# kmjc/PulsePortraiture

Measured on AMD Instinct MI355X. Metric: TOAs/sec (phase+DM fit, 64ch×2048bin fp64) at 1/2/4/8 MI355X, higher is better.
Workload: dtype f64

## Files before the change

pulseportraiture_amd/csrc/ppfit_capi_fit.hip:

```cpp
#include "ppfit_host.hpp"

namespace {

int taylor_lds_moments(ppf_ctx* ctx, int nchan, size_t lds_meta) {
  if (ctx->taylor_static_lds == kUnknown) {
    size_t mx = 0;
    const void* ks[4] = {reinterpret_cast<const void*>(&k_fit_taylor<true, false>),
                         reinterpret_cast<const void*>(&k_fit_taylor<false, false>),
                         reinterpret_cast<const void*>(&k_fit_taylor<true, true>),
                         reinterpret_cast<const void*>(&k_fit_taylor<false, true>)};
    for (const void* k : ks) {
      hipFuncAttributes at;
      if (hipFuncGetAttributes(&at, k) != hipSuccess) return 0;
      mx = std::max(mx, at.sharedSizeBytes);
    }
    ctx->taylor_static_lds = mx;
  }
  const size_t stat = ctx->taylor_static_lds;
  const size_t per_block = (kLdsPerCU / kTaylorBlocksPerCU) & ~(size_t)1023;
  if (per_block <= stat + lds_meta) return 0;
  const size_t nl = (per_block - stat - lds_meta) / ((size_t)nchan * sizeof(double));
  return (int)std::min<size_t>(nl, kMT);
}

int sync_event(ppf_ctx* ctx, size_t i, hipEvent_t* out) {
  while (ctx->sync_events.size() <= i) {
    hipEvent_t e;
    HIPCHK(ctx, hipEventCreateWithFlags(&e, hipEventDisableTiming));
    ctx->sync_events.push_back(e);
  }
  *out = ctx->sync_events[i];
  return PPF_OK;
}


struct FitWorkspace : WsPlan {
  int X, R, sig, dsum, st, acc, wsc, T, G;

  FitWorkspace(int nchan, int NHP, bool taylor, bool wide, int64_t ws_limit, int64_t nsub) {
    const size_t bR = (size_t)NHP * sizeof(double2);
    const size_t bC = (size_t)nchan * sizeof(double);
    X = array((size_t)nchan * NHP * sizeof(double2));
    R = array(bR);
    array(bR);
    sig = array(bC);
    dsum = array(bC);
    st = array(sizeof(SolveState));
    acc = array((size_t)2 * nchan * 10 * sizeof(double));
    wsc = array((size_t)nchan * 8 * sizeof(double));
    T = array(taylor ? (size_t)2 * nchan * kMT * sizeof(double) : 0);
    G = array(wide ? align256(std::max(meta_lds(nchan), xspec_dyn_lds(nchan))) : 0);
    lay_out(nsub, ws_limit, 1024);
  }

  void slice(int sub, SpecArgs& sa, FitArgs& fa) const {
    fa.X = sa.X = at<double2>(X, sub);
    fa.R = sa.R = at<double2>(R, sub);
    fa.sig = sa.sig = at<double>(sig, sub);
    fa.dsum = sa.dsum = at<double>(dsum, sub);
    fa.st = at<SolveState>(st, sub);
    fa.acc = at<double>(acc, sub);
    fa.wsc = at<double>(wsc, sub);
    fa.T = per[T] ? at<double>(T, sub) : nullptr;
    fa.gdyn = sa.gdyn = per[G] ? at<unsigned char>(G, sub) : nullptr;
    fa.gdyn_stride = sa.gdyn_stride = per[G];
  }
};

struct FitLaunch {
  int logN, nbin;
  bool wide;
  size_t lds_meta;
  size_t lds_xspec, lds_guess, lds_taylor, lds_scat;
};


int stage_data(ppf_ctx* ctx, hipStream_t st, int n, const SpecArgs& sa, const FitLaunch& L) {
  const int nbin = L.nbin;
  return timed_on(ctx, PPF_K_DATA_XSPEC, st, [&] {
    if (L.logN < 0) {
      const int nrows = n * sa.nchan, NH = nbin / 2 + 1;
      const double* rows = sa.data + (size_t)sa.sub0 * sa.nchan * nbin;
      const dim3 g((nrows + kGenRows - 1) / kGenRows, (NH + 255) / 256);
      double2* dst = sa.D ? sa.D : sa.X;
      if (sa.spec_mode != PPF_SPEC_USE) {
        if (nbin <= kGenLdsTw)
          hipLaunchKernelGGL(k_dft_rows_mfma<true>, g, dim3(kBlock), dft_mfma_lds(nbin, true), st,
                             rows, dst, nrows, nbin, sa.NHP, sa.tw);
        else
          hipLaunchKernelGGL(k_dft_rows_mfma<false>, g, dim3(kBlock), dft_mfma_lds(nbin, false),
                             st, rows, dst, nrows, nbin, sa.NHP, sa.tw);
      }
      hipLaunchKernelGGL(k_data_post_gen, dim3(n), dim3(kBlock), 0, st, sa, nbin);
    }
    LOGN_SWITCH(L.logN, WIDE_SWITCH(L.wide, hipLaunchKernelGGL((k_data_xspec<LG, WD>), dim3(n),
                                                               dim3(XspecCfg<LG>::WPB * 64),
                                                               L.lds_xspec, st, sa)));
  });
}

int stage_guess(ppf_ctx* ctx, hipStream_t st, int n, const FitArgs& fa, const FitLaunch& L) {
  return timed_on(ctx, PPF_K_GUESS, st, [&] {
    if (fa.guess && fa.guess_wave) hipLaunchKernelGGL(k_guess_w, dim3(n), dim3(64), 0, st, fa);
    hipLaunchKernelGGL(k_guess, dim3(n), dim3(kBlock), fa.guess ? L.lds_guess : 0, st, fa);
  });
}

int stage_moments(ppf_ctx* ctx, hipStream_t st, int n, const FitArgs& fa) {
  if (ctx->opt[PPF_OPT_FUSE_MOMENTS]) return PPF_OK;
  return timed_on(ctx, PPF_K_MOMENTS, st, [&] {
    const dim3 g(n, (fa.nchan + 16 * kWaves - 1) / (16 * kWaves));
    if (fa.Dsp) hipLaunchKernelGGL((k_moments<4, true>), g, dim3(kBlock), 0, st, fa);
    else hipLaunchKernelGGL((k_moments<4, false>), g, dim3(kBlock), 0, st, fa);
  });
}

int stage_taylor(ppf_ctx* ctx, hipStream_t st, int n, const FitArgs& fa, const FitLaunch& L) {
  const bool mom = ctx->opt[PPF_OPT_FUSE_MOMENTS] != 0;
  const dim3 g(n), b(kBlock);
  const size_t lds = L.lds_taylor;
  return timed_on(ctx, PPF_K_FIT_TAYLOR, st, [&] {
    WIDE_SWITCH(L.wide, {
      if (fa.Dsp) {
        if (mom) hipLaunchKernelGGL((k_fit_taylor<true, true, WD>), g, b, lds, st, fa);
        else hipLaunchKernelGGL((k_fit_taylor<false, true, WD>), g, b, lds, st, fa);
      } else {
        if (mom) hipLaunchKernelGGL((k_fit_taylor<true, false, WD>), g, b, lds, st, fa);
        else hipLaunchKernelGGL((k_fit_taylor<false, false, WD>), g, b, lds, st, fa);
      }
    });
  });
}

int stage_post(ppf_ctx* ctx, hipStream_t st, int n, const FitArgs& fa, const FitLaunch& L) {
  return timed_on(ctx, PPF_K_POST, st, [&] {
    if (post_wave_ok(fa)) hipLaunchKernelGGL(k_post_w, dim3(n), dim3(64), L.lds_meta, st, fa);
    WIDE_SWITCH(L.wide, {
      if (!post_wave_ok(fa))
        hipLaunchKernelGGL((k_post<false, WD>), dim3(n), dim3(kBlock), L.lds_meta, st, fa);
      hipLaunchKernelGGL((k_post<true, WD>), dim3(n), dim3(kBlock), L.lds_meta, st, fa);
    });
  });
}

int stage_errs(ppf_ctx* ctx, hipStream_t st, int n, const SpecArgs& sa, double* errs_out) {
  if (!errs_out) return PPF_OK;
  HIPCHK(ctx, hipMemcpyAsync(errs_out + (size_t)sa.sub0 * sa.nchan, sa.sig,
                             (size_t)n * sa.nchan * sizeof(double), hipMemcpyDeviceToDevice, st));
  return PPF_OK;
}

int scat_split_solve(ppf_ctx* ctx, const FitArgs& fa, int nc, int split, size_t lds_scat) {
  const int nchan = fa.nchan;
  double* part = static_cast<double*>(ctx->buf[kSpart].p);
  int* ctrs = reinterpret_cast<int*>(part + (size_t)nc * ((nchan + 7) / 8) * kScatPart);
  HIPCHK(ctx, hipMemsetAsync(ctrs, 0, 2 * sizeof(int), ctx->stream));
  constexpr int kCheck = 4;
  int cur = split;
  const int split_tail = std::max(split, std::min(32, (nchan + 31) / 32));
  hipGraphExec_t gx[2] = {nullptr, nullptr};
  auto graph_for = [&](int sp, hipGraphExec_t* ex) -> int {
    if (*ex) return PPF_OK;
    if (!ctx->stream2)
      HIPCHK(ctx, hipStreamCreateWithFlags(&ctx->stream2, hipStreamNonBlocking));
    hipStream_t cs = ctx->stream2;
    hipGraph_t g = nullptr;
    HIPCHK(ctx, hipStreamBeginCapture(cs, hipStreamCaptureModeThreadLocal));
    for (int k = 0; k < kCheck; ++k) {
      hipLaunchKernelGGL(k_scat_sweep, dim3(nc, sp), dim3(kBlock), lds_scat, cs, fa, part, sp, 0);
      hipLaunchKernelGGL(k_scat_step, dim3(nc), dim3(64), 0, cs, fa, part, 0, ctrs, k & 1);
    }
    HIPCHK(ctx, hipStreamEndCapture(cs, &g));
    const hipError_t e = hipGraphInstantiate(ex, g, nullptr, nullptr, 0);
    (void)hipGraphDestroy(g);
    if (e != hipSuccess)
      return fail(ctx, PPF_ERR_DEVICE, "scattering solve graph: %s", hipGetErrorString(e));
    return PPF_OK;
  };
  struct GraphFree {
    hipGraphExec_t* g;
    hipStream_t st;
    ~GraphFree() {
      if (!g[0] && !g[1]) return;
      (void)hipStreamSynchronize(st);
      for (int i = 0; i < 2; ++i)
        if (g[i]) (void)hipGraphExecDestroy(g[i]);
    }
  } gfree{gx, ctx->stream};
  auto issue = [&](int gi) -> int {
    const int it0 = kCheck * gi;
    if (gi > 0 && ctx->opt[PPF_OPT_SCAT_GRAPH]) {
      hipGraphExec_t* ex = &gx[cur == split ? 0 : 1];
      if (int r = graph_for(cur, ex)) return r;
      if (int r = timed(ctx, PPF_K_SOLVE, [&] { (void)hipGraphLaunch(*ex, ctx->stream); }))
        return r;
    } else {
      for (int k = 0; k < kCheck; ++k) {
        const int init = it0 + k == 0 ? 1 : 0;
        if (int r = timed(ctx, PPF_K_SOLVE, [&] {
              hipLaunchKernelGGL(k_scat_sweep, dim3(nc, cur), dim3(kBlock), lds_scat, ctx->stream,
                                 fa, part, cur, init);
            }))
          return r;
        if (int r = timed(ctx, PPF_K_SOLVE, [&] {
              hipLaunchKernelGGL(k_scat_step, dim3(nc), dim3(64), 0, ctx->stream, fa, part, init,
                                 ctrs, (it0 + k) & 1);
            }))
          return r;
      }
    }
    HIPCHK(ctx, hipMemcpyAsync(ctx->active_h + (gi & 1), ctrs + ((it0 + kCheck - 1) & 1),
                               sizeof(int), hipMemcpyDeviceToHost, ctx->stream));
    HIPCHK(ctx, hipEventRecord(ctx->scat_ev[gi & 1], ctx->stream));
    return PPF_OK;
  };
  const int max_groups = (1001 + kCheck) / kCheck + 1;
  if (int r = issue(0)) return r;
  for (int gi = 0;; ++gi) {
    if (gi + 1 < max_groups)
      if (int r = issue(gi + 1)) return r;
    HIPCHK(ctx, hipEventSynchronize(ctx->scat_ev[gi & 1]));
    const int running = ctx->active_h[gi & 1];
    if (running == 0 || gi + 1 >= max_groups) break;
    if (running < ctx->opt[PPF_OPT_SCAT_TAIL]) cur = split_tail;
  }
  return PPF_OK;
}

bool fit_is_tnc(const ppf_fit_desc* d) {
  return d->method == PPF_METHOD_TNC || d->method == PPF_METHOD_TNC_LEGACY;
}
bool fit_is_exact(const ppf_fit_desc* d) { return (d->solver_flags & PPF_SOLVE_EXACT) != 0; }
bool fit_is_taylor(const ppf_fit_desc* d) {
  return !fit_is_exact(d) && d->method == PPF_METHOD_TRUST_NCG;
}

int check_fit_desc(ppf_ctx* ctx, const ppf_fit_desc* d, const ppf_fit_result* o, int* logN) {
  if (d->nchan <= 0 || d->nchan > PPF_MAX_NCHAN)
    return fail(ctx, PPF_ERR_UNSUPPORTED, "nchan=%d outside [1, %d]", d->nchan, PPF_MAX_NCHAN);
  if (d->nmodel <= 0) return fail(ctx, PPF_ERR_INVALID, "nmodel must be >= 1");
  if (d->method != PPF_METHOD_TRUST_NCG && !fit_is_tnc(d) && d->method != PPF_METHOD_NEWTON_CG)
    return fail(ctx, PPF_ERR_UNSUPPORTED, "Method %d is not implemented.", d->method);
  if (d->method == PPF_METHOD_TNC_LEGACY &&
      !(d->fit_flags[0] && d->fit_flags[1] && !d->fit_flags[2] && !d->fit_flags[3] &&
        !d->fit_flags[4]))
    return fail(ctx, PPF_ERR_INVALID, "legacy TNC fits phase and DM only (fit_flags [1,1,0,0,0])");
  if (d->solver_flags & ~(PPF_SOLVE_EXACT | PPF_SOLVE_EVAL | PPF_GUESS_DIRECT))
    return fail(ctx, PPF_ERR_INVALID, "unknown solver_flags bits 0x%x", d->solver_flags);
  if (!d->data || !d->model || !d->freqs || !d->P || !d->init || !d->nu_fit || !d->nu_out)
    return fail(ctx, PPF_ERR_INVALID, "missing required input pointer");
  if (!o->params || !o->param_errs || !o->nu_out || !o->cov || !o->scales || !o->scale_errs ||
      !o->channel_snrs || !o->chi2 || !o->red_chi2 || !o->snr || !o->nfev || !o->status)
    return fail(ctx, PPF_ERR_INVALID, "missing required output pointer");
  if (d->guess && d->guess_Ns < 2) return fail(ctx, PPF_ERR_INVALID, "guess_Ns must be >= 2");
  if (int r = check_nbin_any(ctx, d->nbin, logN)) return r;
  const int smode = d->spec_mode;
  if (smode != PPF_SPEC_NONE) {
    if (smode != PPF_SPEC_STORE && smode != PPF_SPEC_USE)
      return fail(ctx, PPF_ERR_INVALID, "spec_mode %d: PPF_SPEC_NONE, _STORE or _USE", smode);
    if (!d->spec || !d->spec_sig || !d->spec_dsum || !d->spec_R)
      return fail(ctx, PPF_ERR_INVALID, "spec_mode %d: spec, spec_sig, spec_dsum and spec_R "
                  "are required", smode);
    if (!fit_is_taylor(d) || d->fit_flags[3] || d->fit_flags[4])
      return fail(ctx, PPF_ERR_UNSUPPORTED, "the data-spectrum cache takes phase-family "
                  "trust-ncg fits only (tau and alpha not fitted, not PPF_SOLVE_EXACT)");
  }
  return PPF_OK;
}

void bind_fit_args(const ppf_ctx* ctx, const ppf_fit_desc* d, const ppf_fit_result* o,
                   SpecArgs& sa, FitArgs& fa) {
  const int nbin = d->nbin;
  sa.nchan = fa.nchan = d->nchan;
// ... 224 lines not shown
```

pulseportraiture_amd/csrc/ppfit_device.hpp:

```cpp
#pragma once

#ifndef PPF_NT
#define PPF_NT 1
#endif
#ifndef PPF_EARLY_ROW
#define PPF_EARLY_ROW 1
#endif
#include <hip/hip_runtime.h>
#include <stdint.h>
#include <type_traits>

namespace ppf {

template <int I, int N, class F>
__device__ __forceinline__ void static_for_impl(F&& f) {
  if constexpr (I < N) {
    f(std::integral_constant<int, I>{});
    static_for_impl<I + 1, N>(f);
  }
}
template <int N, class F>
__device__ __forceinline__ void static_for(F&& f) { static_for_impl<0, N>(f); }

constexpr double kDconst = 0x1.03560a9f560aap+12;
constexpr double kPi = 3.141592653589793116;
constexpr double kLn10 = 0x1.26bb1bbb55516p+1;
constexpr int kBlock = 256;
constexpr int kWaves = kBlock / 64;

__device__ __forceinline__ double2 cmk(double x, double y) { return make_double2(x, y); }
__device__ __forceinline__ double2 cadd(double2 a, double2 b) { return cmk(a.x + b.x, a.y + b.y); }
__device__ __forceinline__ double2 csub(double2 a, double2 b) { return cmk(a.x - b.x, a.y - b.y); }
__device__ __forceinline__ double2 cscale(double2 a, double s) { return cmk(a.x * s, a.y * s); }
__device__ __forceinline__ double2 cconj(double2 a) { return cmk(a.x, -a.y); }
__device__ __forceinline__ double2 cmul(double2 a, double2 b) {
  return cmk(fma(a.x, b.x, -a.y * b.y), fma(a.x, b.y, a.y * b.x));
}
__device__ __forceinline__ double2 cmulc(double2 a, double2 b) {
  return cmk(fma(a.x, b.x, a.y * b.y), fma(a.y, b.x, -a.x * b.y));
}
__device__ __forceinline__ double cabs2(double2 a) { return fma(a.x, a.x, a.y * a.y); }

__device__ __forceinline__ double2 turn_phasor(double k, double phi) {
  double t = k * phi;
  double e = fma(k, phi, -t);
  double r = (t - rint(t)) + e;
  double s, c;
  sincospi(2.0 * r, &s, &c);
  return cmk(c, s);
}

template <int CTRL>
__device__ __forceinline__ double dpp_mov(double v) {
  const unsigned long long u = __double_as_longlong(v);
  const int lo = __builtin_amdgcn_mov_dpp((int)(unsigned)u, CTRL, 0xF, 0xF, true);
  const int hi = __builtin_amdgcn_mov_dpp((int)(unsigned)(u >> 32), CTRL, 0xF, 0xF, true);
  return __longlong_as_double((long long)(((unsigned long long)(unsigned)hi << 32) | (unsigned)lo));
}
template <int O>
__device__ __forceinline__ double swap_rows(double v) {
  const unsigned long long u = __double_as_longlong(v);
  unsigned lo = (unsigned)u, hi = (unsigned)(u >> 32);
  if constexpr (O == 16) {
    const auto a = __builtin_amdgcn_permlane16_swap(lo, lo, false, false);
    const auto b = __builtin_amdgcn_permlane16_swap(hi, hi, false, false);
    const bool odd = (threadIdx.x & 16) != 0;
    lo = odd ? a[0] : a[1];
    hi = odd ? b[0] : b[1];
  } else {
    const auto a = __builtin_amdgcn_permlane32_swap(lo, lo, false, false);
    const auto b = __builtin_amdgcn_permlane32_swap(hi, hi, false, false);
    const bool up = (threadIdx.x & 32) != 0;
    lo = up ? a[0] : a[1];
    hi = up ? b[0] : b[1];
  }
  return __longlong_as_double((long long)(((unsigned long long)hi << 32) | lo));
}

__device__ __forceinline__ double group8_sum(double v) {
  v += dpp_mov<0xB1>(v);
  v += dpp_mov<0x4E>(v);
  v += dpp_mov<0x141>(v);
  return v;
}

__device__ __forceinline__ double wave_sum(double v) {
  v = group8_sum(v);
  v += dpp_mov<0x140>(v);
  v += swap_rows<16>(v);
  v += swap_rows<32>(v);
  return v;
}

__device__ __forceinline__ double chan8_sum(double v) {
  v += dpp_mov<0x118>(v);
  v += swap_rows<16>(v);
  v += swap_rows<32>(v);
  return v;
}

__device__ __forceinline__ double wave_max(double v) {
  v = fmax(v, dpp_mov<0xB1>(v));
  v = fmax(v, dpp_mov<0x4E>(v));
  v = fmax(v, dpp_mov<0x141>(v));
  v = fmax(v, dpp_mov<0x140>(v));
  v = fmax(v, swap_rows<16>(v));
  v = fmax(v, swap_rows<32>(v));
  return v;
}

__device__ __forceinline__ double lane0(double v) {
  const unsigned long long u = __double_as_longlong(v);
  const unsigned lo = __builtin_amdgcn_readfirstlane((unsigned)u);
  const unsigned hi = __builtin_amdgcn_readfirstlane((unsigned)(u >> 32));
  return __longlong_as_double((long long)(((unsigned long long)hi << 32) | lo));
}

template <int J>
__device__ __forceinline__ double lane_at(double v) {
  const unsigned long long u = __double_as_longlong(v);
  const unsigned lo = __builtin_amdgcn_readlane((unsigned)u, J);
  const unsigned hi = __builtin_amdgcn_readlane((unsigned)(u >> 32), J);
  return __longlong_as_double((long long)(((unsigned long long)hi << 32) | lo));
}

__device__ __forceinline__ double lane_of(double v, int j) {
  const unsigned long long u = __double_as_longlong(v);
  const unsigned lo = __builtin_amdgcn_readlane((unsigned)u, j);
  const unsigned hi = __builtin_amdgcn_readlane((unsigned)(u >> 32), j);
  return __longlong_as_double((long long)(((unsigned long long)hi << 32) | lo));
}

__device__ __forceinline__ double block_sum(double v, double* red) {
  v = wave_sum(v);
  const int lane = threadIdx.x & 63, w = threadIdx.x >> 6;
  if (lane == 0) red[w] = v;
  __syncthreads();
  double s = 0.0;
#pragma unroll
  for (int i = 0; i < kWaves; ++i) s += red[i];
  __syncthreads();
  return s;
}

struct u32x4 { uint32_t v[4]; };

__device__ __forceinline__ u32x4 philox4x32_10(u32x4 c, uint32_t k0, uint32_t k1) {
#pragma unroll
  for (int r = 0; r < 10; ++r) {
    uint64_t p0 = (uint64_t)0xD2511F53u * c.v[0];
    uint64_t p1 = (uint64_t)0xCD9E8D57u * c.v[2];
    uint32_t hi0 = (uint32_t)(p0 >> 32), lo0 = (uint32_t)p0;
    uint32_t hi1 = (uint32_t)(p1 >> 32), lo1 = (uint32_t)p1;
    u32x4 n;
    n.v[0] = hi1 ^ c.v[1] ^ k0;
    n.v[1] = lo1;
    n.v[2] = hi0 ^ c.v[3] ^ k1;
    n.v[3] = lo0;
    c = n;
// ... 471 lines not shown
```

pulseportraiture_amd/csrc/ppfit_kernels.hpp:

```cpp
#pragma once
#include "ppfit.h"
#include "ppfit_device.hpp"
#include "ppfit_rowfft.hpp"

namespace ppf {

struct SpecArgs {
  int sub0, nchan, NHP, kc, guess;
  int log10_tau, fit_tau, exact;
  int spec_mode;
  const double* data;
  const double2* M;
  const int* model_idx;
  const double* freqs;
  const double* errs;
  const uint8_t* mask;
  const double* weights;
  const double* P;
  const double* init;
  const double* guess_nu;
  double2* X;
  double2* R;
  double* sig;
  double* dsum;
  const double2* tw;
  double2* D;
  unsigned char* gdyn;
  size_t gdyn_stride;
};

template <bool WIDE, class Args>
__device__ __forceinline__ unsigned char* chan_tables(const Args& a, unsigned char* lds) {
  if constexpr (WIDE) return a.gdyn + (size_t)blockIdx.x * a.gdyn_stride;
  else return lds;
}

__device__ __forceinline__ bool spec_taylor_sub(const SpecArgs& a, int s) {
  const double t3 = a.init[(size_t)s * 5 + 3];
  const double tl = a.log10_tau ? pow(10.0, t3) : t3;
  return !a.exact && !a.fit_tau && tl == 0.0;
}

struct PhaseShiftArgs {
  int NHP, kc, Ns;
  double lo, hi;
  const double* data;
  const double2* M;
  const int* model_idx;
  const double* noise;
  double* out;
  const double2* tw;
};

struct NbScatArgs {
  int nprof, nbin, NH, kc;
  int log10_tau;
  const double2* D;
  const double2* M;
  const int* model_idx;
  const double* noise;
  const double* tau0;
  double* out;
  int* status;
  int* nfev;
};

constexpr int kMT = 32;
__host__ __device__ constexpr int kVpowRows(int N) { return N + 1 + 4 * 64; }
constexpr int kMTerm = kMT - 2;
constexpr size_t kLdsPerCU = 160 * 1024;
constexpr int kTaylorBlocksPerCU = 3;
constexpr double kTaylorY = 3.0;

struct SolveState {
  double x[5];
  double init[5];
  double fun;
  double refs[3];
  int nfev, status;
  int slot;
  int scat;
  int scat_post;
  int taylor;
  double xc[2][5];
  int mvalid, xslot;
  double g[5], H[25], tr;
  double xp[5], pl[5], predv;
  int hits, kit, sdone;
};

struct FitArgs {
  int sub0, nchan, nbin, NH, NHP, kc;
  int flags[5];
  int log10_tau, option, is_toa, guess, Ns, guess_wrap;
  int solver_flags;
  int method;
  int guess_wave;
  int post_wave;
  const double2* X;
  const double2* Dsp;
  const double2* R;
  const double2* M;
  const double* M2;
  const double* pn;
  const int* model_idx;
  const double* sig;
  const double* dsum;
  const double* freqs;
  const uint8_t* mask;
  const double* P;
  const double* init;
  const double* nu_fit;
  const double* nu_out;
  const double* guess_nu;
  const double* guess_tau;
  SolveState* st;
  double* T;
  int tlds;
  int tnl;
  const double2* tw;
  const double2* vpow;
  const double2* Mmean;
  unsigned long long* ptime;
  double* trace;
  int trace_cap;
  double* acc;
  double* wsc;
  double* o_params;
  double* o_param_errs;
  double* o_nu_out;
  double* o_cov;
  double* o_scales;
  double* o_scale_errs;
  double* o_channel_snrs;
  double* o_chi2;
  double* o_red_chi2;
  double* o_snr;
  int* o_nfev;
  int* o_status;
  double* o_init_used;
  double* o_fun;
  double* o_cov_nosc;
  double* o_grad;
  double* o_hess;
  double bounds[5][2];
  unsigned char* gdyn;
  size_t gdyn_stride;
};

#ifndef PPF_POST_WAVE_NCHAN
#define PPF_POST_WAVE_NCHAN 128
#endif
constexpr int kPostWaveNchan = PPF_POST_WAVE_NCHAN;
__host__ __device__ inline bool post_wave_ok(const FitArgs& a) {
  return a.post_wave && a.T && a.nchan <= kPostWaveNchan && !a.flags[3] && !a.flags[4];
}

constexpr int kTraceRec = 32;
__device__ __forceinline__ void trace_sweep(const FitArgs& a, int s, int isweep, const double* x,
                                            const double* out, int nout, bool counted) {
  if (!a.trace || threadIdx.x != 0 || isweep >= a.trace_cap) return;
  double* r = a.trace + ((size_t)s * a.trace_cap + isweep) * kTraceRec;
  for (int i = 0; i < 5; ++i) r[i] = x[i];
  for (int i = 0; i < 21; ++i) r[5 + i] = i < nout ? out[i] : NAN;
  r[26] = counted ? 1.0 : 0.0;
  r[27] = (double)isweep;
}

struct GuessShared {
  double red[kWaves];
  double bestv[kWaves];
  int besti[kWaves];
  double x0, x, fx;
  double out[8];
  double bf[kBlock];
  double2 fb[kBlock / 2];
  double2 fw[kBlock / 2];
  double ev[2][kWaves];
};

__device__ __forceinline__ bool argmin_better(double v, int i, double bv, int bi) {
  if (i == 0x7fffffff) return false;
  if (bi == 0x7fffffff) return true;
  if (isnan(bv)) return isnan(v) && i < bi;
  if (isnan(v)) return true;
  return v < bv || (v == bv && i < bi);
}

__device__ __forceinline__ double row_eval_phase(const double2* rm, int k0, int k1, double phi) {
  const double2 z = turn_phasor(1.0, phi);
  double acc = 0.0;
  for (int kb = k0; kb < k1; kb += 64) {
    double2 e = turn_phasor((double)kb, phi);
    const int ke = min(kb + 64, k1);
#pragma unroll 4
    for (int k = kb; k < ke; ++k) {
      const double2 r = rm[k];
      acc = fma(r.x, e.x, acc);
      acc = fma(-r.y, e.y, acc);
      e = cmul(e, z);
    }
  }
  return acc;
}

__device__ __forceinline__ double block_eval_phase(const double2* rm, int NH, double phi,
                                                   double* slot) {
  const int tid = threadIdx.x, lane = tid & 63, w = tid >> 6;
  const double2 st = turn_phasor((double)kBlock, phi);
  double2 e = turn_phasor((double)tid, phi);
  double acc = 0.0;
  for (int k = tid; k < NH; k += kBlock) {
    const double2 r = rm[k];
    acc = fma(r.x, e.x, acc);
    acc = fma(-r.y, e.y, acc);
    e = cmul(e, st);
  }
  acc = wave_sum(acc);
  if (lane == 0) slot[w] = acc;
  __syncthreads();
  double t = slot[0];
#pragma unroll
  for (int q = 1; q < kWaves; ++q) t += slot[q];
  return t;
// ... 586 lines not shown
```

pulseportraiture_amd/csrc/ppfit_taylor.hip:

```cpp
#include "ppfit_kernels.hpp"

namespace ppf {

template <int NH>
__device__ __forceinline__ void rs_step(const double* v, double* out, int o, bool upper) {
#pragma unroll
  for (int i = 0; i < NH; ++i) {
    const double keep = upper ? v[NH + i] : v[i];
    const double send = upper ? v[i] : v[NH + i];
    out[i] = keep + __shfl_xor(send, o);
  }
}

template <int O>
__device__ __forceinline__ double pair_swap_sum(double lo, double hi) {
  const unsigned long long a = __double_as_longlong(lo), b = __double_as_longlong(hi);
  unsigned a0 = (unsigned)a, a1 = (unsigned)(a >> 32), b0 = (unsigned)b, b1 = (unsigned)(b >> 32);
  if constexpr (O == 32) {
    const auto r0 = __builtin_amdgcn_permlane32_swap(a0, b0, false, false);
    const auto r1 = __builtin_amdgcn_permlane32_swap(a1, b1, false, false);
    a0 = r0[0]; b0 = r0[1]; a1 = r1[0]; b1 = r1[1];
  } else {
    static_assert(O == 16, "permlane swaps exist for 16 and 32");
    const auto r0 = __builtin_amdgcn_permlane16_swap(a0, b0, false, false);
    const auto r1 = __builtin_amdgcn_permlane16_swap(a1, b1, false, false);
    a0 = r0[0]; b0 = r0[1]; a1 = r1[0]; b1 = r1[1];
  }
  return __longlong_as_double((long long)(((unsigned long long)a1 << 32) | a0)) +
         __longlong_as_double((long long)(((unsigned long long)b1 << 32) | b0));
}
template <int NH, int O>
__device__ __forceinline__ void rs_swap(const double* v, double* out) {
#pragma unroll
  for (int i = 0; i < NH; ++i) out[i] = pair_swap_sum<O>(v[i], v[NH + i]);
}

typedef double f64x4 __attribute__((ext_vector_type(4)));

constexpr int kMomReseedSteps = 8;
#ifndef PPF_DSP_U
#define PPF_DSP_U 2
#endif
#ifndef PPF_MOM_U
#define PPF_MOM_U 4
#endif


__device__ __forceinline__ double2 xload(const double2* p) { return *p; }

__device__ __forceinline__ double vpow_m(double v, double v2, double v4, double v8, int m) {
  double pc = (m & 1) ? v : 1.0;
  pc *= (m & 2) ? v2 : 1.0;
  pc *= (m & 4) ? v4 : 1.0;
  pc *= (m & 8) ? v8 : 1.0;
  return (m & 16) ? pc * (v8 * v8) : pc;
}

__device__ __forceinline__ double2 vpow_inline(int k, double iN, int col) {
  const double v = (double)k * iN;
  const double v2 = v * v, v4 = v2 * v2, v8 = v4 * v4;
  return cmk(vpow_m(v, v2, v4, v8, 2 * col), vpow_m(v, v2, v4, v8, 2 * col + 1));
}

__global__ void k_vpow(double2* vp, int nbin, int rows) {
  const int i = blockIdx.x * blockDim.x + threadIdx.x;
  if (i >= rows * 16) return;
  const int k = i >> 4, col = i & 15;
  vp[i] = vpow_inline(k, 2.0 / (double)nbin, col);
}

template <int U, bool DSP>
__device__ __forceinline__ void moment_tile16(const FitArgs& a, int c, int slot, int n, bool ok,
                                              double phic) {
  static_assert(kMT == 32, "two 16-row MFMA tiles");
  static_assert(U % 2 == 0, "steps go in pairs");
  constexpr int UP = U / 2;
  const int lane = threadIdx.x & 63;
  const int N = a.nbin / 2;
  const int nblk = ((N + 1 + 3) / 4 + U - 1) / U;
  const int col = lane & 15, kk = lane >> 4;
  const size_t xrow = ((size_t)c * a.nchan + (ok ? n : 0)) * a.NHP;
  const double2* __restrict__ Xr = (DSP ? a.Dsp : a.X) + xrow;
  const double2* __restrict__ Mr = nullptr;
  if constexpr (DSP) {
    const int s = a.sub0 + c;
    const int midx = a.model_idx ? a.model_idx[s] : 0;
    Mr = a.M + ((size_t)midx * a.nchan + (ok ? n : 0)) * a.NHP;
  }
  const double2* __restrict__ vp = a.vpow + (size_t)kk * 16 + col;
  const double2 s8 = turn_phasor(8.0, phic);
  f64x4 d0 = {0.0, 0.0, 0.0, 0.0}, d2 = d0;
  f64x4 g0 = d0, g2 = d0;
  double2 xb[U], pb[U], mb[DSP ? U : 1];
#pragma unroll
  for (int t = 0; t < U; ++t) {
    xb[t] = xload(Xr + min(4 * t + kk, N));
    if constexpr (DSP) mb[t] = Mr[min(4 * t + kk, N)];
    pb[t] = vp[(size_t)t * 64];
  }
  auto xcell = [&](int t, int i) {
    const int k = 4 * t + kk;
    if constexpr (DSP) {
      const double2 x = cmulc(xb[i], mb[i]);
      return (ok && k >= 1 && k <= N) ? x : cmk(0.0, 0.0);
    } else {
      return (ok && k <= N) ? xb[i] : cmk(0.0, 0.0);
    }
  };
  double2 e0 = cmk(1.0, 0.0), e1 = e0;
  for (int b = 0; b < nblk; ++b) {
    if ((b * U) % kMomReseedSteps == 0) {
      e0 = turn_phasor((double)(4 * (b * U) + kk), phic);
      e1 = turn_phasor((double)(4 * (b * U + 1) + kk), phic);
    }
#pragma unroll
    for (int u = 0; u < UP; ++u) {
      const double2 W0 = cmul(xcell(b * U + 2 * u, 2 * u), e0);
      const double2 W1 = cmul(xcell(b * U + 2 * u + 1, 2 * u + 1), e1);
      const double2 p0 = pb[2 * u], p1 = pb[2 * u + 1];
      d0 = __builtin_amdgcn_mfma_f64_16x16x4f64(p0.x, W0.x, d0, 0, 0, 0);
      g0 = __builtin_amdgcn_mfma_f64_16x16x4f64(p0.y, W0.y, g0, 0, 0, 0);
      d2 = __builtin_amdgcn_mfma_f64_16x16x4f64(p1.x, W1.x, d2, 0, 0, 0);
      g2 = __builtin_amdgcn_mfma_f64_16x16x4f64(p1.y, W1.y, g2, 0, 0, 0);
      e0 = cmul(e0, s8);
      e1 = cmul(e1, s8);
#pragma unroll
      for (int h = 0; h < 2; ++h) {
        const int t = 2 * u + h;
        xb[t] = xload(Xr + min(4 * ((b + 1) * U + t) + kk, N));
        if constexpr (DSP) mb[t] = Mr[min(4 * ((b + 1) * U + t) + kk, N)];
        pb[t] = vp[(size_t)((b + 1) * U + t) * 64];
      }
    }
  }
  d0 += d2;
  g0 += g2;
  if (ok) {
    double2* Tn = reinterpret_cast<double2*>(a.T + (((size_t)c * 2 + slot) * a.nchan + n) * kMT);
#pragma unroll
    for (int r = 0; r < 4; ++r) Tn[kk + 4 * r] = cmk(d0[r], g0[r]);
  }
}

template <int U, bool DSP>
__device__ __forceinline__ void moment_tile8(const FitArgs& a, int c, int slot, int n, bool ok,
                                             double phic) {
  static_assert(kMT == 32, "two 16-row MFMA tiles");
  static_assert(U % 2 == 0, "steps go in pairs");
  constexpr int UP = U / 2;
  const int lane = threadIdx.x & 63;
  const int N = a.nbin / 2;
  const int nblk = ((N + 1 + 3) / 4 + U - 1) / U;
  const int col = lane & 15, part = col & 1, kk = lane >> 4;
  const size_t xrow = ((size_t)c * a.nchan + (ok ? n : 0)) * a.NHP;
  const double2* __restrict__ Xr = (DSP ? a.Dsp : a.X) + xrow;
  const double2* __restrict__ Mr = nullptr;
  if constexpr (DSP) {
    const int s = a.sub0 + c;
    const int midx = a.model_idx ? a.model_idx[s] : 0;
    Mr = a.M + ((size_t)midx * a.nchan + (ok ? n : 0)) * a.NHP;
  }
  auto xget = [&](bool on, int k) {
    if constexpr (DSP) return (on && k >= 1 && k <= N) ? cmulc(Xr[k], Mr[k]) : cmk(0.0, 0.0);
    else return (on && k <= N) ? Xr[k] : cmk(0.0, 0.0);
  };
  const double2 s8 = turn_phasor(8.0, phic);
  const double iN = 2.0 / (double)a.nbin;
  f64x4 d0 = {0.0, 0.0, 0.0, 0.0}, d1 = d0, d2 = d0, d3 = d0;
  double2 xb[UP];
#pragma unroll
  for (int u = 0; u < UP; ++u) {
    const int k = 4 * (2 * u + part) + kk;
    xb[u] = xget(ok, k);
  }
  double2 e = cmk(1.0, 0.0);
  for (int b = 0; b < nblk; ++b) {
    const bool more = b + 1 < nblk;
    if ((b * U) % kMomReseedSteps == 0) e = turn_phasor((double)(4 * (b * U + part) + kk), phic);
#pragma unroll
    for (int u = 0; u < UP; ++u) {
      const double2 W = cmul(xb[u], e);
      const double recv = dpp_mov<0xB1>(part ? W.x : W.y);
      const double bv0 = part ? recv : W.x;
      const double bv1 = part ? W.y : recv;
      const double2 p0 = vpow_inline(4 * (b * U + 2 * u) + kk, iN, col);
      const double2 p1 = vpow_inline(4 * (b * U + 2 * u + 1) + kk, iN, col);
      d0 = __builtin_amdgcn_mfma_f64_16x16x4f64(p0.x, bv0, d0, 0, 0, 0);
      d1 = __builtin_amdgcn_mfma_f64_16x16x4f64(p0.y, bv0, d1, 0, 0, 0);
      d2 = __builtin_amdgcn_mfma_f64_16x16x4f64(p1.x, bv1, d2, 0, 0, 0);
      d3 = __builtin_amdgcn_mfma_f64_16x16x4f64(p1.y, bv1, d3, 0, 0, 0);
      e = cmul(e, s8);
      const int k = 4 * ((b + 1) * U + 2 * u + part) + kk;
      xb[u] = xget(more && ok, k);
    }
  }
  d0 += d2;
  d1 += d3;
  if (ok) {
    double* Tn = a.T + (((size_t)c * 2 + slot) * a.nchan + n) * kMT;
#pragma unroll
    for (int r = 0; r < 4; ++r) Tn[2 * (kk + 4 * r) + part] = part ? d1[r] : d0[r];
  }
}

template <bool DSP>
__device__ void moments_from_X(const FitArgs& a, const Meta& m, int c, int s, int slot,
                               const double* xc, const double* refs, double P) {
  const int lane = threadIdx.x & 63, w = threadIdx.x >> 6;
  const int chl = (lane & 15) >> 1;
  for (int t = w; t * 8 < m.nok; t += kWaves) {
    const int j = t * 8 + chl;
    const bool ok = j < m.nok;
    moment_tile8<DSP ? 4 : 8, DSP>(a, c, slot, ok ? m.chan[j] : 0, ok,
                    ok ? phase_frac(xc, m.fr[j], refs, P) : 0.0);
  }
}

template <int U, bool DSP>
__global__ __launch_bounds__(kBlock, 3) void k_moments(FitArgs a) {
  const int c = blockIdx.x, s = a.sub0 + c;
  if (!fused_taylor(a, s)) return;
  const int lane = threadIdx.x & 63, w = threadIdx.x >> 6;
  const int n0 = 16 * (kWaves * (int)blockIdx.y + w);
  if (n0 >= a.nchan) return;
  const SolveState& st = a.st[c];
  const int n = n0 + (lane & 15);
  const bool ok = n < a.nchan && (!a.mask || a.mask[(size_t)s * a.nchan + n]);
  const double phic = ok ? phase_frac(st.xc[0], a.freqs[(size_t)s * a.nchan + n], st.refs, a.P[s])
                         : 0.0;
  moment_tile16<U, DSP>(a, c, 0, n, ok, phic);
}

template __global__ void k_moments<4, false>(FitArgs);
template __global__ void k_moments<4, true>(FitArgs);

struct TaylorShared {
  double x[5], xp[5];
  double xc[2][5];
  double out[48];
  double red[kWaves][48];
  double ifact[kMT];
  int done, nok, slot, tslot, q, mvalid;
  int same;
  TrustNcgLds sv;
};

__device__ __forceinline__ void stage_T0(const FitArgs& a, int c, double* tl) {
  const double* __restrict__ src = a.T + (size_t)c * 2 * a.nchan * kMT;
  const int nl = a.tnl;
  const int n = a.nchan * nl;
  constexpr int kU = 8;
  for (int i0 = 0; i0 < n; i0 += kBlock * kU) {
    double v[kU];
#pragma unroll
    for (int u = 0; u < kU; ++u) {
      const int i = i0 + u * kBlock + (int)threadIdx.x;
      const int ch = i / nl;
      v[u] = i < n ? src[(size_t)ch * kMT + (i - ch * nl)] : 0.0;
    }
#pragma unroll
    for (int u = 0; u < kU; ++u) {
      const int i = i0 + u * kBlock + (int)threadIdx.x;
      if (i < n) tl[i] = v[u];
    }
  }
}

__device__ __forceinline__ double wave_reach(const Meta& m, double p0, double p1, double p2,
                                             const double* xc, double Ks) {
  const double prm[3] = {p0, p1, p2};
  double mx = 0.0;
  for (int j = (int)threadIdx.x & 63; j < m.nok; j += 64)
    mx = fmax(mx, fabs(taylor_delta_lin(prm, xc, m.d1[j], m.d2[j])));
  return kTwoPi * Ks * wave_max(mx);
}


template <bool MOM, bool DSP, bool WIDE>
__global__ __launch_bounds__(kBlock, 3) void k_fit_taylor(FitArgs a) {
  extern __shared__ __align__(16) unsigned char dyn[];
  __shared__ TaylorShared sh;
  __shared__ double refs[3];
  const int c = blockIdx.x, s = a.sub0 + c, tid = threadIdx.x;
  const int lane = tid & 63;
  if (!fused_taylor(a, s)) return;
  const bool prof = a.ptime != nullptr;
  unsigned long long t0 = prof ? wall_clock64() : 0ull;
  auto mark = [&](int i) {
    if (prof) {
      const unsigned long long t1 = wall_clock64();
      if (tid == 0) atomicAdd(&a.ptime[i], t1 - t0);
      t0 = t1;
    }
  };
  if constexpr (MOM) {
    const SolveState& st0 = a.st[c];
    const int w = tid >> 6;
    for (int t = w; 16 * t < a.nchan; t += kWaves) {
      const int n = 16 * t + (lane & 15);
      const bool ok = n < a.nchan && (!a.mask || a.mask[(size_t)s * a.nchan + n]);
      const double phic =
          ok ? phase_frac(st0.xc[0], a.freqs[(size_t)s * a.nchan + n], st0.refs, a.P[s]) : 0.0;
      moment_tile16<DSP ? PPF_DSP_U : PPF_MOM_U, DSP>(a, c, 0, n, ok, phic);
    }
    __builtin_amdgcn_fence(__ATOMIC_RELEASE, "workgroup");
    __syncthreads();
    __builtin_amdgcn_fence(__ATOMIC_ACQUIRE, "workgroup");
  }
  mark(0);
  unsigned char* dmeta = chan_tables<WIDE>(a, dyn);
  SolveState& st = a.st[c];
  double* tl = a.tlds ? reinterpret_cast<double*>(dyn + a.tlds) : nullptr;
  if (tl) stage_T0(a, c, tl);
  const Meta m = load_meta(a, c, s, dmeta, &sh.nok);
  const double P = a.P[s];
  const double Ks = 0.5 * (double)a.nbin;
  if (tid < 5) sh.x[tid] = st.x[tid];
  if (tid < 5) sh.xc[0][tid] = st.xc[0][tid];
  if (tid < 3) refs[tid] = st.refs[tid];
  if (tid < kMT) sh.ifact[tid] = c_inv_fact[tid];
  if (tid == 0) {
    sh.done = (m.nok == 0);
    sh.slot = 0;
    sh.tslot = 0;
    sh.mvalid = 1;
    st.mvalid = 1;
  }
  __syncthreads();
  mark(1);
  double* acc0 = a.acc + (size_t)c * 2 * a.nchan * NACC;
  TrustNcg tn;
  auto pick = [&](double p0, double p1, double p2) -> int {
    int best = -1;
    double by = INFINITY;
    for (int q = 0; q < 2; ++q) {
      if (!(sh.mvalid & (1 << q))) continue;
      const double y = wave_reach(m, p0, p1, p2, sh.xc[q], Ks);
      if (y <= kTaylorY && y < by) { by = y; best = q; }
    }
    return best;
  };
  auto source = [&](int q) {
    const bool l = q == 0 && tl;
    return TaylorSrc{a.T + ((size_t)c * 2 + q) * a.nchan * kMT, sh.xc[q], refs, true, sh.ifact,
                     l ? tl : nullptr, l ? a.tnl : 0};
  };
  auto recentre = [&](const double* p) -> int {
    const int wsl = sh.tslot ^ 1;
    if (prof && tid == 0) atomicAdd(&a.ptime[8], 1ull);
    if (tid == 0) {
      st.mvalid &= ~(1 << wsl);
      sh.mvalid = st.mvalid;
      for (int i = 0; i < 5; ++i) st.xc[wsl][i] = p[i];
    }
    if (tid < 5) sh.xc[wsl][tid] = p[tid];
    __syncthreads();
    moments_from_X<DSP>(a, m, c, s, wsl, sh.xc[wsl], refs, P);
    __syncthreads();
    if (wsl == 0 && tl) stage_T0(a, c, tl);
    if (tid == 0) {
      st.mvalid |= 1 << wsl;
      sh.mvalid = st.mvalid;
    }
    __syncthreads();
    if (tid < 64) {
      const int q = pick(p[0], p[1], p[2]);
      if (lane == 0) sh.q = q;
    }
    __syncthreads();
    return sh.q;
  };
  if (!sh.done) {
    if (tid < 64) {
      const int q0 = pick(sh.x[0], sh.x[1], sh.x[2]);
      if (lane == 0) sh.q = q0;
    }
    __syncthreads();
    int q = sh.q;
    if (q < 0) q = recentre(sh.x);
    mark(2);
    sweep<0, false>(a, m, c, s, sh.x, refs, P, acc0, sh.out, sh.red, source(q));
    mark(3);
    if (tid == 0) sh.tslot = q;
  }
  if (tid < 64) {
    const bool done =
        tn.start(sh.out, sh.x, lane, m.nok, (a.solver_flags & PPF_SOLVE_EVAL) != 0);
    if (m.nok) trace_sweep(a, s, 0, sh.x, sh.out, 21, true);
    if (lane == 0 && done) sh.done = 1;
    tn.park(sh.sv, lane);
  }
  __syncthreads();
  while (!sh.done) {
    if (tid < 64) {
      tn.unpark(sh.sv, lane);
      bool same = false;
      const bool go = tn.propose(lane, same);
      if (go) {
        const double pv = tn.xl + tn.pl;
        if (lane < 5) sh.xp[lane] = pv;
        const int qp = same ? sh.q : pick(__shfl(pv, 0), __shfl(pv, 1), __shfl(pv, 2));
        if (lane == 0) {
          sh.q = qp;
          sh.same = same;
        }
      } else if (lane == 0) {
        sh.done = 1;
      }
      tn.park(sh.sv, lane);
    }
    __syncthreads();
    mark(4);
    if (sh.done) break;
    const bool fresh = !sh.same;
    int q = sh.q;
    if (fresh && q < 0) q = recentre(sh.xp);
    mark(2);
    double* sl = acc0 + (size_t)(sh.slot ^ 1) * a.nchan * NACC;
    if (fresh) sweep<0, false>(a, m, c, s, sh.xp, refs, P, sl, sh.out, sh.red, source(q));
    mark(3);
    if (tid < 64) {
      tn.unpark(sh.sv, lane);
      bool accepted;
      const bool done = tn.judge(sh.out, lane, fresh, accepted);
      if (fresh) trace_sweep(a, s, tn.nfev - 1, sh.xp, sh.out, 21, true);
      if (lane == 0) {
        if (accepted) { sh.slot ^= 1; sh.tslot = q; }
        if (done) sh.done = 1;
      }
      tn.park(sh.sv, lane);
    }
    __syncthreads();
  }
  if (tid < 64) {
    tn.unpark(sh.sv, lane);
    tn.finish(a, st, s, lane, m.nok, sh.slot, false);
  }
  if (tid == 0) {
    st.xslot = sh.tslot;
    if (prof) atomicAdd(&a.ptime[9], 1ull);
  }
}

template __global__ void k_fit_taylor<false, false>(FitArgs);
template __global__ void k_fit_taylor<true, false>(FitArgs);
template __global__ void k_fit_taylor<false, true>(FitArgs);
template __global__ void k_fit_taylor<true, true>(FitArgs);
template __global__ void k_fit_taylor<false, false, true>(FitArgs);
template __global__ void k_fit_taylor<true, false, true>(FitArgs);
template __global__ void k_fit_taylor<false, true, true>(FitArgs);
template __global__ void k_fit_taylor<true, true, true>(FitArgs);

__global__ void k_selftest(int* fails) {
  const int l = threadIdx.x & 63;
  const double x = (double)l;
  auto chk = [&](int t, bool ok) { if (!ok) atomicAdd(&fails[t], 1); };
// ... 30 lines not shown
```

Measured before the change: 1.312 million.

## Stage fused moment loads through LDS transpose for coalesced global reads

Adds a staged variant of the fused moment tile for the non-Dsp path. Each wave loads a 16-channel by 16-harmonic block with coalesced global reads, writes it to an XOR-swizzled per-wave LDS buffer, and reads it back transposed to feed the f64 MFMA accumulation. The next block is prefetched while the current one is computed. The aim is to replace strided per-channel global loads with coalesced ones. In exchange it adds LDS traffic, may raise dynamic LDS use, and relies on intra-wave ordering with no explicit barrier.

After: 1.351 million (median of 6 runs). 1.03x the previous value.

```diff
diff --git a/pulseportraiture_amd/csrc/ppfit_capi_fit.hip b/pulseportraiture_amd/csrc/ppfit_capi_fit.hip
--- a/pulseportraiture_amd/csrc/ppfit_capi_fit.hip
+++ b/pulseportraiture_amd/csrc/ppfit_capi_fit.hip
@@ -118,7 +118,8 @@
 int stage_taylor(ppf_ctx* ctx, hipStream_t st, int n, const FitArgs& fa, const FitLaunch& L) {
   const bool mom = ctx->opt[PPF_OPT_FUSE_MOMENTS] != 0;
   const dim3 g(n), b(kBlock);
-  const size_t lds = L.lds_taylor;
+  const bool stage = PPF_MOM_STAGE && mom && !fa.Dsp;
+  const size_t lds = stage ? std::max(L.lds_taylor, kWaves * kMomStageBytes) : L.lds_taylor;
   return timed_on(ctx, PPF_K_FIT_TAYLOR, st, [&] {
     WIDE_SWITCH(L.wide, {
       if (fa.Dsp) {
diff --git a/pulseportraiture_amd/csrc/ppfit_device.hpp b/pulseportraiture_amd/csrc/ppfit_device.hpp
--- a/pulseportraiture_amd/csrc/ppfit_device.hpp
+++ b/pulseportraiture_amd/csrc/ppfit_device.hpp
@@ -5,6 +5,9 @@
 #endif
 #ifndef PPF_EARLY_ROW
 #define PPF_EARLY_ROW 1
+#endif
+#ifndef PPF_MOM_STAGE
+#define PPF_MOM_STAGE 1
 #endif
 #include <hip/hip_runtime.h>
 #include <stdint.h>
diff --git a/pulseportraiture_amd/csrc/ppfit_kernels.hpp b/pulseportraiture_amd/csrc/ppfit_kernels.hpp
--- a/pulseportraiture_amd/csrc/ppfit_kernels.hpp
+++ b/pulseportraiture_amd/csrc/ppfit_kernels.hpp
@@ -70,6 +70,7 @@
 constexpr int kMTerm = kMT - 2;
 constexpr size_t kLdsPerCU = 160 * 1024;
 constexpr int kTaylorBlocksPerCU = 3;
+constexpr size_t kMomStageBytes = 16 * 16 * 16;
 constexpr double kTaylorY = 3.0;
 
 struct SolveState {
diff --git a/pulseportraiture_amd/csrc/ppfit_taylor.hip b/pulseportraiture_amd/csrc/ppfit_taylor.hip
--- a/pulseportraiture_amd/csrc/ppfit_taylor.hip
+++ b/pulseportraiture_amd/csrc/ppfit_taylor.hip
@@ -142,6 +142,84 @@
   }
 }
 
+__device__ __forceinline__ void moment_tile16_staged(const FitArgs& a, int c, int n0, int n,
+                                                     bool ok, double phic, double2* buf) {
+  static_assert(kMT == 32, "two 16-row MFMA tiles");
+  constexpr int U = 4;
+  static_assert(kMomStageBytes == 16 * 4 * U * sizeof(double2), "one block of U steps");
+  static_assert(kMomReseedSteps % U == 0, "re-seeds fall on block starts");
+  const int lane = threadIdx.x & 63;
+  const int N = a.nbin / 2;
+  const int nblk = (N + 1 + 15) / 16;
+  const int col = lane & 15, kk = lane >> 4;
+  const double2* __restrict__ Xc = a.X + (size_t)c * a.nchan * a.NHP;
+  unsigned goff[U];
+  int wr[U], rd[U];
+#pragma unroll
+  for (int j = 0; j < U; ++j) {
+    const int ch = 4 * j + kk;
+    goff[j] = (unsigned)min(n0 + ch, a.nchan - 1) * (unsigned)a.NHP + (unsigned)col;
+    wr[j] = 16 * ch + (col ^ ch);
+    rd[j] = 16 * col + ((4 * j + kk) ^ col);
+  }
+  const double2* __restrict__ vp = a.vpow + (size_t)kk * 16 + col;
+  const double2 s8 = turn_phasor(8.0, phic);
+  f64x4 d0 = {0.0, 0.0, 0.0, 0.0}, d2 = d0;
+  f64x4 g0 = d0, g2 = d0;
+  double2 xs[U], pb[U];
+#pragma unroll
+  for (int j = 0; j < U; ++j) xs[j] = xload(Xc + goff[j]);
+#pragma unroll
+  for (int t = 0; t < U; ++t) pb[t] = vp[(size_t)t * 64];
+  double2 e0 = cmk(1.0, 0.0), e1 = e0;
+  for (int b = 0; b < nblk; ++b) {
+    if ((b * U) % kMomReseedSteps == 0) {
+      e0 = turn_phasor((double)(4 * (b * U) + kk), phic);
+      e1 = turn_phasor((double)(4 * (b * U + 1) + kk), phic);
+    }
+#pragma unroll
+    for (int j = 0; j < U; ++j) buf[wr[j]] = xs[j];
+    const unsigned bn = 16u * (unsigned)min(b + 1, nblk - 1);
+#pragma unroll
+    for (int j = 0; j < U; ++j) xs[j] = xload(Xc + goff[j] + bn);
+    __builtin_amdgcn_sched_barrier(0);
+    double2 xr[U];
+#pragma unroll
+    for (int t = 0; t < U; ++t) xr[t] = buf[rd[t]];
+    asm volatile("" : "+v"(xr[0].x), "+v"(xr[0].y), "+v"(xr[1].x), "+v"(xr[1].y),
+                      "+v"(xr[2].x), "+v"(xr[2].y), "+v"(xr[3].x), "+v"(xr[3].y));
+#pragma unroll
+    for (int t = 0; t < U; ++t) {
+      const bool on = ok & (4 * (b * U + t) + kk <= N);
+      xr[t] = cmk(on ? xr[t].x : 0.0, on ? xr[t].y : 0.0);
+    }
+#pragma unroll
+    for (int u = 0; u < U / 2; ++u) {
+      const double2 W0 = cmul(xr[2 * u], e0);
+      const double2 W1 = cmul(xr[2 * u + 1], e1);
+      const double2 p0 = pb[2 * u], p1 = pb[2 * u + 1];
+      d0 = __builtin_amdgcn_mfma_f64_16x16x4f64(p0.x, W0.x, d0, 0, 0, 0);
+      g0 = __builtin_amdgcn_mfma_f64_16x16x4f64(p0.y, W0.y, g0, 0, 0, 0);
+      d2 = __builtin_amdgcn_mfma_f64_16x16x4f64(p1.x, W1.x, d2, 0, 0, 0);
+      g2 = __builtin_amdgcn_mfma_f64_16x16x4f64(p1.y, W1.y, g2, 0, 0, 0);
+      e0 = cmul(e0, s8);
+      e1 = cmul(e1, s8);
+#pragma unroll
+      for (int h = 0; h < 2; ++h) {
+        const int t = 2 * u + h;
+        pb[t] = vp[(size_t)((b + 1) * U + t) * 64];
+      }
+    }
+  }
+  d0 += d2;
+  g0 += g2;
+  if (ok) {
+    double2* Tn = reinterpret_cast<double2*>(a.T + ((size_t)c * 2 * a.nchan + n) * kMT);
+#pragma unroll
+    for (int r = 0; r < 4; ++r) Tn[kk + 4 * r] = cmk(d0[r], g0[r]);
+  }
+}
+
 template <int U, bool DSP>
 __device__ __forceinline__ void moment_tile8(const FitArgs& a, int c, int slot, int n, bool ok,
                                              double phic) {
@@ -301,7 +379,11 @@
       const bool ok = n < a.nchan && (!a.mask || a.mask[(size_t)s * a.nchan + n]);
       const double phic =
           ok ? phase_frac(st0.xc[0], a.freqs[(size_t)s * a.nchan + n], st0.refs, a.P[s]) : 0.0;
-      moment_tile16<DSP ? PPF_DSP_U : PPF_MOM_U, DSP>(a, c, 0, n, ok, phic);
+      if constexpr (!DSP && PPF_MOM_STAGE)
+        moment_tile16_staged(a, c, 16 * t, n, ok, phic,
+                             reinterpret_cast<double2*>(dyn + (size_t)w * kMomStageBytes));
+      else
+        moment_tile16<DSP ? PPF_DSP_U : PPF_MOM_U, DSP>(a, c, 0, n, ok, phic);
     }
     __builtin_amdgcn_fence(__ATOMIC_RELEASE, "workgroup");
     __syncthreads();
```
